# jdryg/vg-renderer

Measured on AMD Instinct MI355X. Metric: M tessellated verts/sec (stroke+fill AA), Tiger×10k batch, 1/2/4/8 GPUs, higher is better.
Workload: dtype f32; 1 GPU; tiger-like 240-path drawing (seed 2024) x 10000 instances per GPU: convexFillAA on every sub-path + polylineStrokeAA/AAThin (Butt/Miter) on 1/3 of the paths; instances_per_gpu=10000, draws_per_gpu=2400000, parallelism=shard1, verts_per_gpu=414940000, indices_per_gpu=1816170000, meshes_per_gpu=4350000, poly_verts_per_gpu=140430000

## Files before the change

### vg-renderer_amd/csrc/vgx_api.hip

```cpp
#include "vgx_internal.h"
#include "vgx_scan.h"
#include "vgx_scan_ops.h"
#include "vgx_pathsim.h"
#include "vgx_inst.h"
#include "vgx_flat1.h"
#include "vgx_thin.h"
#include "vgx_pathset_dev.h"
#include "vgx_tile.h"
#include "vgx_mscan.h"
#include "vgx_dash.h"
#include "vgx_update.h"
#include "vgx_raster.h"
#include "vgx_damage.h"
#include "vgx_pick.h"
#include "vgx_concave_lane.h"
#include "vgx_scratch.h"
#include <vector>
#include <algorithm>
#include <atomic>
#include <string.h>
#include <math.h>
#include <new>
#include <stdlib.h>

// ... 27 lines not shown
{
	T* host;
	uint32_t n;
	hipEvent_t ev;
	bool pending;
	int create(vgx_ctx* ctx, uint32_t count);
	void push(vgx_ctx* ctx, const void* dev, hipStream_t s);
	bool landed();
	void release();
};

struct VgxGatherWire { vgx_rank_sizes z; uint64_t chunk; };

struct VgxTemplateState
{
	bool on;
	bool isBatch;
	const vgx_pathset* ps;
	uint64_t psGen;
	uint32_t period;
	uint32_t classes;
	VgxTmplKernel kernel;
	uint32_t tileSize;
	vgx_sizes inst;
	vgx_sizes total;
	uint64_t numWg, nDraws;
	uint32_t round;
	uint32_t roundElems;
	uint32_t roundLds;
	uint64_t relemWords;
};
struct VgxTemplate : VgxTemplateState
{
	Buf<VgxTmplTile> tile;
	Buf<float2> poly; Buf<VgxTmplMesh> mesh; Buf<vgx_mesh> mtab; Buf<VgxTmplElem> elem; Buf<vgx_draw> draws;
	Buf<unsigned long long> hash, clsSum; Buf<uint32_t> instCls, clsRep; Buf<VgxTmplClass> cls; Buf<VgxTmplInst> iinfo; Buf<uint2> wg;
	Buf<VgxTmplRoundMesh> trmesh; Buf<uint2> tmsz;
	Buf<unsigned long long> rsz, itot, iplace; Buf<uint2> relem; Buf<VgxTmplMeshPlace> mplace;
};
static_assert(sizeof(VgxTmplWg) == sizeof(uint2) && offsetof(VgxTmplWg, inst) == offsetof(uint2, x) && offsetof(VgxTmplWg, tile) == offsetof(uint2, y), "the host's workgroup table is uploaded as uint2");
static_assert(sizeof(VgxTmplClass) == 40 && offsetof(VgxTmplClass, round) == 32 && sizeof(VgxTmplClass().round) == 8, "VgxTmplClass: the named words lie where the padding did");
static_assert(sizeof(VgxTmplMesh) == 64 && offsetof(VgxTmplMesh, fringe_bits) == 56 && offsetof(VgxTmplMesh, round_no) == 60, "VgxTmplMesh: the named words lie where the padding did");

struct vgx_ctx
{
	int device;
	int lastHipError;
	int pendingHipError;
	DevBufList scratch;
	Buf<uint32_t> asmJump0, asmJump1, asmStart, meshBase;
	vgx_assembly asmCfg;
	bool asmArmed;
	Buf<uint64_t> subPrefix;
	DevBuf cmdPrefix;
	DevBuf poly;
	DevBuf partial;
	Buf<uint32_t> cmdCnt, serialList;
	Buf<VgxSubRec> subFirst;
	Buf<float> leafOverflow;
// ... 1392 lines not shown
	if ((st = ensure(ctx, ctx->tmpl.relem, (classes ? ctx->tmpl.relemWords : n * a.num_round_elems) + 1)) != VGX_OK) { return st; }
	if ((st = ensure(ctx, ctx->tmpl.mplace, (classes ? a.total.num_meshes : n * a.inst.num_meshes) + 1)) != VGX_OK) { return st; }
	if ((st = ensure(ctx, ctx->partial, VGX_SCAN_BLOCKS * sizeof(Sum3))) != VGX_OK) { return st; }
	a.rsz = classes ? nullptr : ctx->tmpl.rsz.ptr(); a.relem = ctx->tmpl.relem.ptr();
	a.mplace = ctx->tmpl.mplace.ptr();
	if (vgx_tmpl_round_per_instance(a)) {
		if ((st = ensure(ctx, ctx->tmpl.itot, (n + 1) * 2)) != VGX_OK) { return st; }
		if ((st = ensure(ctx, ctx->tmpl.iplace, (n + 1) * 2)) != VGX_OK) { return st; }
		a.itot = ctx->tmpl.itot.ptr(); a.iplace = ctx->tmpl.iplace.ptr();
	}
	vgx_launch_tmpl_round_sizes(a, (Sum3*)ctx->partial.p, s);
	mark(ctx, s, "tmpl_round_sizes");
	return VGX_OK;
}

static void tmplArgs(vgx_ctx* ctx, const vgx_pathset* ps, const vgx_draw* draws, uint64_t ndraws, VgxTmplArgs& a)
{
	a.draws = draws; a.ndraws = ndraws; a.period = ctx->tmpl.period; a.ninst = ndraws / ctx->tmpl.period; a.npaths = ps->dev.npaths;
	a.tdraws = ctx->tmpl.draws.ptr(); a.tpoly = ctx->tmpl.poly.ptr(); a.tmesh = ctx->tmpl.mesh.ptr();
	a.tmtab = ctx->tmpl.mtab.ptr(); a.telem = ctx->tmpl.elem.ptr();
	a.inst = ctx->tmpl.inst;
	a.ttile = ctx->tmpl.tile.ptr();
	a.tile = ctx->tmpl.tileSize;
	a.tiles_per_inst = (uint32_t)((ctx->tmpl.inst.num_elements + a.tile - 1) / a.tile);
	a.caps = ctx->caps;
	a.totals = ctx->totals.ptr();
	a.kernel = ctx->tmpl.kernel;
	if (ctx->tmpl.classes > 1) {
		a.iinfo = ctx->tmpl.iinfo.ptr(); a.wg = ctx->tmpl.wg.ptr(); a.num_wg = ctx->tmpl.numWg;
		a.cls = ctx->tmpl.cls.ptr(); a.round_lds = ctx->tmpl.roundLds;
		a.total = ctx->tmpl.total;
	} else {
		memset(&a.total, 0, sizeof(a.total));
		vgx_tmpl_add_instances(a.total, a.ninst, ctx->tmpl.inst);
		a.num_wg = a.ninst * (uint64_t)a.tiles_per_inst;
	}
}

static int runTmpl(vgx_ctx* ctx, const vgx_pathset* ps, const vgx_draw* draws, uint64_t ndraws, const vgx_mesh_out* out, vgx_sizes* dev_sizes, uint32_t* dev_status, hipStream_t s)
{
	VgxTmplArgs a;
	memset(&a, 0, sizeof(a));
	tmplArgs(ctx, ps, draws, ndraws, a);
	a.pos = out->pos; a.color = out->color; a.idx = out->idx; a.meshes_out = out->meshes;
	a.caps.vertices = out->cap_vertices; a.caps.indices = out->cap_indices; a.caps.meshes = out->cap_meshes;
	if (a.num_wg > 0x7FFFFFFFull) { return VGX_E_RANGE; }
	noteHip(ctx, hipMemsetAsync(ctx->totals.p, 0, sizeof(VgxTotals), s));
// ... 157 lines not shown
	noteHip(ctx, hipMemsetAsync(ctx->tmpl.cls.p, 0, ((size_t)T + 1) * sizeof(VgxTmplClass), j.s));
	if (general) {
		j.b.mdesc = ctx->mdesc.ptr(); j.b.num_meshes = j.all.num_meshes; j.b.nclasses = T; j.b.cls = ctx->tmpl.cls.ptr();
		vgx_launch_tmpl_styles(j.b, j.s);
		HIPCHK(ctx, hipMemcpyAsync(&styles, &VGX_TMPL_STYLES(ctx->tmpl.cls.ptr(), T), sizeof(uint32_t), hipMemcpyDeviceToHost, j.s));
		HIPCHK(ctx, hipStreamSynchronize(j.s));
	}
	j.t.kernel = vgx_tmpl_kernel_for(styles);
	j.t.tileSize = vgx_tmpl_tile_for(j.t.kernel, ctx->optTmplTile);
	return VGX_OK;
}

static TmplStage tmplBuildTables(TmplJob& j)
{
	vgx_ctx* ctx = j.ctx;
	const uint32_t T = j.T;
	const uint64_t M = j.all.num_meshes, V = j.all.num_poly_vertices;
	VgxTmplBuild& b = j.b;
	int st;
	b.draws = ctx->tmpl.draws.ptr(); b.poly = (const float2*)ctx->poly.p; b.mdesc = ctx->mdesc.ptr(); b.mprep = ctx->mprep.ptr(); b.mtab = ctx->mtab.ptr();
	b.prefix_fill = ctx->elemPrefix.ptr(); b.prefix_stroke = ctx->elemPrefixS.ptr();
	b.num_meshes = M; b.num_elems = j.all.num_elements; b.tile = j.t.tileSize; b.period = (uint32_t)j.P; b.nclasses = T;
	b.num_vertices = j.all.num_vertices; b.num_indices = j.all.num_indices; b.cls = ctx->tmpl.cls.ptr();
	vgx_launch_tmpl_classes(b, j.s);
	j.cls.resize((size_t)T + 1);
	std::vector<unsigned long long> csum(((size_t)T + 1) * 5, 0ull);
	if (T > 1) {
		if ((st = ensure(ctx, ctx->tmpl.clsSum, ((size_t)T + 1) * 5)) != VGX_OK) { return st; }
		vgx_launch_tmpl_class_sums(b, ctx->dinfo.ptr(), (const uint64_t*)ctx->cmdPrefix.p, j.P * T, j.all, ctx->tmpl.clsSum.ptr(), j.s);
		HIPCHK(ctx, hipMemcpyAsync(csum.data(), ctx->tmpl.clsSum.p, csum.size() * sizeof(unsigned long long), hipMemcpyDeviceToHost, j.s));
	}
	HIPCHK(ctx, hipMemcpyAsync(j.cls.data(), ctx->tmpl.cls.p, ((size_t)T + 1) * sizeof(VgxTmplClass), hipMemcpyDeviceToHost, j.s));
	HIPCHK(ctx, hipStreamSynchronize(j.s));
	if (T > 1 && !vgx_tmpl_class_sizes(j.cls.data(), csum.data(), T, j.csz)) { return TMPL_ORDINARY; }
	const uint64_t tiles = j.cls[T].tile0;
	if ((st = ensure(ctx, ctx->tmpl.poly, V + 1)) != VGX_OK) { return st; }
	if ((st = ensure(ctx, ctx->tmpl.mesh, M + 1)) != VGX_OK) { return st; }
	if ((st = ensure(ctx, ctx->tmpl.mtab, M + 1)) != VGX_OK) { return st; }
	if ((st = ensure(ctx, ctx->tmpl.elem, tiles * j.t.tileSize + 64)) != VGX_OK) { return st; }
	if ((st = ensure(ctx, ctx->tmpl.tile, tiles + 1)) != VGX_OK) { return st; }
	if ((st = ensure(ctx, ctx->tmpl.trmesh, M + 2)) != VGX_OK) { return st; }
	if ((st = ensure(ctx, ctx->tmpl.tmsz, M + 1)) != VGX_OK) { return st; }
	if ((st = ensure(ctx, ctx->partial, VGX_SCAN_BLOCKS * sizeof(Sum3))) != VGX_OK) { return st; }
	b.tmsz = ctx->tmpl.tmsz.ptr(); b.trmesh = ctx->tmpl.trmesh.ptr();
	b.has_round = vgx_tmpl_kernel_is_round(j.t.kernel) ? 1u : 0u;
	b.partial = (Sum3*)ctx->partial.p;
	b.ttile = ctx->tmpl.tile.ptr();
	b.tmesh = ctx->tmpl.mesh.ptr(); b.tmtab = ctx->tmpl.mtab.ptr(); b.telem = ctx->tmpl.elem.ptr();
	vgx_launch_tmpl_build(b, j.s);
	HIPCHK(ctx, hipMemcpyAsync(ctx->tmpl.poly.p, ctx->poly.p, V * 2 * sizeof(float), hipMemcpyDeviceToDevice, j.s));
	return VGX_OK;
}

static TmplStage tmplReadRoundLayout(TmplJob& j)
{
	vgx_ctx* ctx = j.ctx;
	const uint32_t T = j.T;
	j.clsRelems.assign(T, 0);
// ... 1609 lines not shown
```

### vg-renderer_amd/csrc/vgx_internal.h

```cpp
#ifndef VGX_INTERNAL_H
#define VGX_INTERNAL_H

#include <hip/hip_runtime.h>
#include <stdint.h>
#include "../../include/vgx.h"
#include "vgx_lane.h"

#include "vgx_internal_types.h"
#include "vgx_tmpl_plan.h"

struct VgxFlattenArgs
{
	VgxPathSetDev ps;
	const vgx_draw* draws;
	uint64_t ndraws;
	const uint64_t* cmd_prefix;
	const uint64_t* sub_prefix;
	uint32_t* cmd_cnt;
	vgx_draw_info* dinfo;
	float* poly;
	vgx_subpath* subs;
	VgxMeshDesc* mdesc;
	VgxMeshPrep* mprep;
	vgx_mesh* mtab;
// ... 31 lines not shown
	vgx_mesh* meshes_out;
	const uint32_t* mesh_base;
	VgxTotals* totals;
	VgxCaps caps;
	int no_long;
	int tile_mode;
};


#ifndef VGX_TMPL_THREADS
#define VGX_TMPL_THREADS 512
#endif
struct VgxTmplBuild
{
	const vgx_draw* draws;
	const VgxMeshDesc* mdesc;
	const VgxMeshPrep* mprep;
	const vgx_mesh* mtab;
	const float2* poly;
	const uint64_t* prefix_fill;
	const uint64_t* prefix_stroke;
	uint64_t num_meshes, num_elems;
	uint32_t tile;
	VgxTmplMesh* tmesh;
	vgx_mesh* tmtab;
	VgxTmplElem* telem;
	VgxTmplTile* ttile;
	uint32_t period;
	uint32_t nclasses;
	uint64_t num_vertices, num_indices;
	VgxTmplClass* cls;
	VgxTmplRoundMesh* trmesh;
	uint2* tmsz;
	uint32_t has_round;
	struct Sum3* partial;
};
struct VgxTmplArgs
{
	const vgx_draw* draws;
	uint64_t ndraws;
	uint64_t ninst;
	uint32_t period;
	uint32_t npaths;
	const vgx_draw* tdraws;
	const float2* tpoly;
	const VgxTmplMesh* tmesh;
// ... 406 lines not shown
```

### vg-renderer_amd/csrc/vgx_tmpl.hip

```cpp
#include <stddef.h>
#include <type_traits>
#include "vgx_internal.h"
#include "vgx_wave.h"
#include "vgx_elem.h"
#include "vgx_tmpl_elem.h"
#include "vgx_scan_ops.h"

namespace {

static_assert(sizeof(vgx_draw) == 64 && offsetof(vgx_draw, path) == 0 && offsetof(vgx_draw, fill_flags) == 4 && offsetof(vgx_draw, fill_color) == 8
	&& offsetof(vgx_draw, stroke_flags) == 12 && offsetof(vgx_draw, stroke_color) == 16 && offsetof(vgx_draw, stroke_width) == 20 && offsetof(vgx_draw, scale) == 24
	&& offsetof(vgx_draw, tess_tol) == 28 && offsetof(vgx_draw, fringe) == 32 && offsetof(vgx_draw, mtx) == 36, "draw records are read as four 16-byte words");
__device__ __forceinline__ bool tmpl_same(const uint4 a0, const uint4 a1, const uint4 a2, const uint4 b0, const uint4 b1, const uint4 b2)
{
	return ((a0.x == b0.x) & (a0.y == b0.y) & (a0.w == b0.w) & (a1.y == b1.y) & (a1.z == b1.z) & (a1.w == b1.w) & (a2.x == b2.x)) != 0;
}

__device__ __forceinline__ uint32_t tmpl_validate(const uint4 q0, const uint4 q1, const uint4 q2, const uint4 q3, uint32_t npaths)
{
	const uint32_t sf = q0.w;
	if (q0.x >= npaths || ((sf & VGX_STROKE_ENABLE) && (VGX_STROKE_CAP(sf) > 2u || VGX_STROKE_JOIN(sf) > 2u))) { return VGX_E_INVALID_ARG; }
	const float sw = __uint_as_float(q1.y), sc = __uint_as_float(q1.z), tt = __uint_as_float(q1.w), fr = __uint_as_float(q2.x);
	const float m0 = __uint_as_float(q2.y), m1 = __uint_as_float(q2.z), m2 = __uint_as_float(q2.w);
	const float m3 = __uint_as_float(q3.x), m4 = __uint_as_float(q3.y), m5 = __uint_as_float(q3.z);
// ... 43 lines not shown
{
	for (uint64_t i = (uint64_t)blockIdx.x * blockDim.x + threadIdx.x; i < ndraws; i += (uint64_t)gridDim.x * blockDim.x) {
		const uint4* q = (const uint4*)(draws + i);
		const uint4 q0 = q[0], q1 = q[1], q2 = q[2];
		const uint64_t inst = i / P;
		unsigned long long h = tmpl_mix(0x243F6A8885A308D3ull, (uint32_t)(i - inst * P));
		h = tmpl_mix(h, q0.x); h = tmpl_mix(h, q0.y); h = tmpl_mix(h, q0.w); h = tmpl_mix(h, q1.y); h = tmpl_mix(h, q1.z); h = tmpl_mix(h, q1.w); h = tmpl_mix(h, q2.x);
		atomicAdd(&hashes[inst], h);
	}
}
__global__ __launch_bounds__(256) void k_tmpl_check_cls(const vgx_draw* draws, uint64_t ndraws, uint64_t P, const uint32_t* inst_cls, const uint32_t* cls_rep, VgxTotals* totals)
{
	bool bad = false;
	for (uint64_t i = (uint64_t)blockIdx.x * blockDim.x + threadIdx.x; i < ndraws; i += (uint64_t)gridDim.x * blockDim.x) {
		const uint64_t inst = i / P;
		const uint64_t k = i - inst * P;
		const uint4* q = (const uint4*)(draws + i);
		const uint4* t = (const uint4*)(draws + (uint64_t)cls_rep[inst_cls[inst]] * P + k);
		bad = bad || !tmpl_same(q[0], q[1], q[2], t[0], t[1], t[2]);
	}
	if (bad) { totals->tmpl_bad = 1u; }
}

__global__ void k_tmpl_classes(VgxTmplBuild B)
{
	const uint64_t M = B.num_meshes;
	uint32_t tile0 = 0;
	for (uint32_t c = 0; c <= B.nclasses; ++c) {
		uint64_t lo = 0, hi = M;
		const uint64_t d0 = (uint64_t)c * B.period;
		while (lo < hi) {
			const uint64_t mid = (lo + hi) >> 1;
			if (B.mdesc[mid].draw < d0) { lo = mid + 1; } else { hi = mid; }
		}
		VgxTmplClass r;
		r.mesh0 = (uint32_t)lo;
		r.elem0 = B.prefix_fill[lo] + B.prefix_stroke[lo];
		r.v0 = lo < M ? B.mtab[lo].first_vertex : B.num_vertices;
		r.i0 = lo < M ? B.mtab[lo].first_index : B.num_indices;
		r.tile0 = tile0;
		r.round[VGX_TC_ELEM0] = B.cls[c].round[VGX_TC_ELEM0]; r.round[VGX_TC_MESH0] = 0;
		B.cls[c] = r;
		if (c > 0) {
			const uint64_t e = r.elem0 - B.cls[c - 1].elem0;
			B.cls[c].tile0 = B.cls[c - 1].tile0 + (uint32_t)((e + B.tile - 1) / B.tile);
		}
		tile0 = B.cls[c].tile0;
	}
}
__global__ __launch_bounds__(256) void k_tmpl_class_sums(VgxTmplBuild B, const vgx_draw_info* dinfo, const uint64_t* cmdPrefix, uint64_t numDraws, vgx_sizes all, unsigned long long* sums)
{
	__shared__ unsigned long long s_serial;
	const uint32_t c = blockIdx.x;
	const uint64_t d0 = (uint64_t)c * B.period;
	if (threadIdx.x == 0) { s_serial = 0ull; }
	__syncthreads();
	if (c > 0) {
		unsigned long long n = 0;
		for (uint64_t d = d0 - B.period + threadIdx.x; d < d0; d += 256) { n += (dinfo[d].flags & 1u) ? 1ull : 0ull; }
		if (n) { atomicAdd(&s_serial, n); }
	}
	__syncthreads();
	if (threadIdx.x == 0) {
		unsigned long long* o = sums + 5ull * c;
		const bool end = d0 >= numDraws;
		o[0] = end ? all.num_poly_vertices : dinfo[d0].first_poly_vertex;
		o[1] = end ? all.num_subpaths : dinfo[d0].first_subpath;
		o[2] = cmdPrefix[end ? numDraws : d0];
// ... 114 lines not shown
	__shared__ unsigned long long s_poly[VGX_TMPL_ELEMS_MAXM];
	__shared__ uint32_t s_pick;
	__shared__ uint64_t s_b[6];
	auto lastLe = [&](uint64_t x, uint64_t lo, uint64_t hi) {
		while (hi - lo > 1) {
			const uint64_t step = (hi - lo + 255) / 256;
			const uint64_t m = lo + (uint64_t)tid * step;
			if (tid == 0) { s_pick = 0; }
			__syncthreads();
			if (tid > 0 && m < hi && first(m) <= x) { atomicMax(&s_pick, tid); }
			__syncthreads();
			const uint32_t k = s_pick;
			__syncthreads();
			lo += (uint64_t)k * step;
			hi = lo + step < hi ? lo + step : hi;
		}
		return lo;
	};
	for (uint64_t tile = blockIdx.x; tile < B.cls[B.nclasses].tile0; tile += gridDim.x) {
		uint32_t c = 0;
		while (c + 1 < B.nclasses && B.cls[c + 1].tile0 <= tile) { ++c; }
		const VgxTmplClass cl = B.cls[c];
		const uint64_t cEnd = B.cls[c + 1].elem0;
		const uint64_t x0 = cl.elem0 + (tile - cl.tile0) * T;
		const uint64_t x1 = x0 + T < cEnd ? x0 + T : cEnd;
		const uint64_t m0 = lastLe(x0, 0, M);
		const uint64_t m1 = x1 >= E ? M : lastLe(x1, m0, (m0 + T / 2 + 2 < M) ? m0 + T / 2 + 2 : M);
		const uint64_t hi = m1 < M ? m1 + 1 : M;
		const bool inLds = hi - m0 <= (uint64_t)VGX_TMPL_ELEMS_MAXM;
		__syncthreads();
		if (inLds) {
			for (uint64_t m = m0 + tid; m < hi; m += 256) {
				const VgxMeshDesc md = B.mdesc[m];
				s_pf[m - m0] = B.prefix_fill[m];
				s_ps[m - m0] = B.prefix_stroke[m] | (VGX_MD_KIND(md.kind) < VGX_MESH_STROKE ? (1ull << 63) : 0ull);
				s_poly[m - m0] = md.poly_first;
			}
		}
		if (tid == 0) {
			auto before = [&](uint64_t x, uint64_t m, uint64_t* fB, uint64_t* sB, uint32_t* j) {
				if (m >= M) { *fB = B.prefix_fill[M]; *sB = B.prefix_stroke[M]; *j = 0; return; }
				const uint64_t pf = B.prefix_fill[m], psk = B.prefix_stroke[m];
				const uint32_t jj = (uint32_t)(x - (pf + psk));
				const bool f = VGX_MD_KIND(B.mdesc[m].kind) < VGX_MESH_STROKE;
				*j = jj; *fB = pf + (f ? jj : 0u); *sB = psk + (f ? 0u : jj);
			};
			uint64_t f0, s0, f1, s1;
			uint32_t j0, j1;
			before(x0, m0, &f0, &s0, &j0);
			before(x1, x1 >= E ? M : m1, &f1, &s1, &j1);
// ... 230 lines not shown
	uint32_t cmesh0;
	const vgx_draw* tdraws;
};
__device__ __forceinline__ void tmpl_mesh_out(const VgxTmplArgs& A, const TmplPlace& P, uint32_t mesh)
{
	vgx_mesh mr = A.tmtab[mesh];
	mr.first_vertex += P.v;
	mr.first_index += P.i;
	mr.draw += P.draw0;
	A.meshes_out[P.m + (mesh - P.cmesh0)] = mr;
}

__device__ __forceinline__ void tmpl_mesh_out_placed(const VgxTmplArgs& A, const TmplPlace& P, uint32_t mesh, uint4 mi)
{
	vgx_mesh mr = A.tmtab[mesh];
	mr.first_vertex = P.v + mi.x;
	mr.first_index = P.i + mi.y;
	mr.num_vertices = mi.z;
	mr.num_indices = mi.w;
	mr.draw += P.draw0;
	A.meshes_out[P.m + (mesh - P.cmesh0)] = mr;
}

struct TmplVtx01
{
	float x0, y0, x1, y1;
	__device__ __forceinline__ V2 ld(uint32_t i) const { const bool z = i == 0; return v2(z ? x0 : x1, z ? y0 : y1); }
};

__device__ __forceinline__ void tmpl_stroke_counts(uint32_t kind, uint32_t cap, uint32_t join, uint32_t H, uint32_t* capNv, uint32_t* capNiFirst, uint32_t* joinNv, uint32_t* joinNi, uint32_t* bridge)
{
	const uint32_t R = (kind == VGX_MESH_STROKE) ? 2u : (kind == VGX_MESH_STROKE_AA ? 4u : 3u);
	*bridge = (R - 1) * 6;
	const bool roundCap = cap == VGX_CAP_ROUND && kind != VGX_MESH_STROKE_AA_THIN;
	if (roundCap) {
		*capNv = kind == VGX_MESH_STROKE_AA ? 2 * H : H;
		*capNiFirst = kind == VGX_MESH_STROKE_AA ? 9 * H - 12 : 3 * (H - 2);
	} else {
		*capNv = R;
		*capNiFirst = kind == VGX_MESH_STROKE_AA ? 6u : 0u;
	}
	if (kind == VGX_MESH_STROKE_AA_THIN) { const bool bevel = join != VGX_JOIN_MITER; *joinNv = bevel ? 4u : 3u; *joinNi = bevel ? 3u : 0u; }
	else if (join == VGX_JOIN_MITER) { *joinNv = R; *joinNi = 0; }
	else if (kind == VGX_MESH_STROKE_AA) { *joinNv = 6; *joinNi = 9; }
	else { *joinNv = 3; *joinNi = 3; }
}
// ... 298 lines not shown
	}
}
#ifndef VGX_TMPL_OCC
#define VGX_TMPL_OCC
#endif
#ifndef VGX_TMPL_G_THREADS
#define VGX_TMPL_G_THREADS 256
#endif
#define VGX_TMPL_G_TILE VGX_TMPL_GENERAL_TILE
template<int KIND, int THREADS, int MAXTILE, int ROUND = 0>
__device__ __forceinline__ void tmpl_emit_body(const VgxTmplArgs& A)
{
	constexpr bool GENERAL = KIND == 2;
	static_assert(ROUND == 0 || GENERAL || KIND == 3 || KIND == 4, "Round joins take the general element body, or -- closed AA strokes only -- tmpl_stroke_elem_round");
	constexpr int CH = MAXTILE / THREADS;
	__shared__ TmplDraw s_draw[VGX_TMPL_MAXM];
	__shared__ TmplRec s_rec[VGX_TMPL_MAXM];
	__shared__ float2 s_vtx[MAXTILE];
	__shared__ float2 s_dir[MAXTILE];
	__shared__ uint32_t s_status;
	__shared__ uint4 s_mi[ROUND ? VGX_TMPL_MAXM : 1];
	__shared__ float4 s_rmesh[ROUND ? VGX_TMPL_MAXM : 1];
	__shared__ float s_fringe[KIND >= 2 ? VGX_TMPL_MAXM : 1];
	const uint32_t tid = threadIdx.x;
	uint32_t inst32, t;
	TmplPlace P;
	uint64_t relemAt = 0;
	if (A.wg) {
		const uint2 w = A.wg[blockIdx.x];
		inst32 = w.x; t = w.y;
		const VgxTmplInst ii = A.iinfo[inst32];
		P.v = ii.v; P.i = ii.i; P.m = ii.m;
		if (ROUND) { P.v = A.iplace[2 * (uint64_t)inst32]; P.i = A.iplace[2 * (uint64_t)inst32 + 1]; relemAt = ii.rel; }
	} else {
		inst32 = blockIdx.x / A.tiles_per_inst;
		t = blockIdx.x - inst32 * A.tiles_per_inst;
		P.v = (uint64_t)inst32 * A.inst.num_vertices; P.i = (uint64_t)inst32 * A.inst.num_indices; P.m = (uint64_t)inst32 * A.inst.num_meshes;
		if (ROUND) {
			if (A.iplace) { P.v = A.iplace[2 * (uint64_t)inst32]; P.i = A.iplace[2 * (uint64_t)inst32 + 1]; }
			else { const VgxTmplMeshPlace* mp = A.mplace + (uint64_t)inst32 * A.inst.num_meshes; P.v = mp->v; P.i = mp->i; }
			relemAt = (uint64_t)inst32 * A.num_round_elems;
		}
	}
	const uint64_t inst = inst32;
	const VgxTmplTile tl = A.ttile[t];
	P.draw0 = (uint32_t)(inst * A.period); P.cmesh0 = tl.cmesh0; P.tdraws = A.tdraws + tl.cdraw0;
// ... 53 lines not shown
			} else if (j == 0 && A.meshes_out) { tmpl_mesh_out(A, P, er.mesh); }
			const uint32_t ibase = meshBase ? meshBase[er.mesh - P.cmesh0] : 0u;
			tmpl_elem_emit<KIND, 0>(O, j, tm.kind, N, vOff, iOff, ibase, kind < VGX_MESH_STROKE ? dr.fill_color : dr.stroke_color, f0, tm.f1, tmpl_xf(xf, vt[j]), dir(j), dir, vtx,
				__uint_as_float(tm.fringe_bits), P.tdraws + tm.drawk, A.tmesh + er.mesh, rpl);
		}
		return;
	}
#ifdef VGX_TMPL_PROFILE
	const unsigned long long tp0 = wall_clock64();
#define TMPL_PROF(i) do { if (tid == 0) { atomicAdd(&A.totals->prof[i], wall_clock64() - tp0); } } while (0)
#else
#define TMPL_PROF(i)
#endif
	if (ROUND && tid < nm) { s_mi[tid] = minfoOf(mA + tid); }
	VgxTmplElem er[CH];
	uint32_t rb[ROUND ? CH : 1], rk[ROUND ? CH : 1];
#pragma unroll
	for (int c = 0; c < CH; ++c) {
		const uint32_t s = (uint32_t)c * THREADS + tid;
		er[c].mesh = mA; er[c].jq = 0; er[c].lx = 0.0f; er[c].ly = 0.0f;
		if (s < nel) { er[c] = telem[s]; }
	}
	VgxTmplMesh tm;
	memset(&tm, 0, sizeof(tm));
	tm.n = 3; tm.drawk = dA; tm.kind = VGX_MESH_FILL;
	uint32_t ibase = 0;
	uint4 mi = make_uint4(0u, 0u, 0u, 0u);
	if (tid < nm) {
		tm = A.tmesh[mA + tid];
		if (meshBase) { ibase = meshBase[mA - P.cmesh0 + tid]; }
	}
	if (tid < nd) { s_draw[tid] = tmpl_load_draw(A, idraws, P.tdraws, dA + tid); }
	if (tid == 0) { s_status = A.totals->status; }
	__syncthreads();
	const uint32_t status = s_status;
	if (tid < nm) {
		if (ROUND) { mi = s_mi[tid]; tm.v_off = mi.x; tm.i_off = mi.y; }
		const uint32_t kind = VGX_MD_KIND(tm.kind);
		const TmplDraw* d = &s_draw[tm.drawk - dA];
		TmplRec r;
		r.ibase = ibase; r.n = tm.n; r.v_off = tm.v_off; r.i_off = tm.i_off;
		r.kind = (tm.kind & 0xFFFFu) | ((tm.drawk - dA) << 16); r.color = kind < VGX_MESH_STROKE ? d->fill_color : d->stroke_color; r.f0 = tm.f0; r.f1 = tm.f1;
		if (KIND >= 2) { s_fringe[tid] = __uint_as_float(tm.fringe_bits); }
		if (ROUND) {
			const bool rj = tm.round_no != 0;
			s_rmesh[tid] = make_float4(__uint_as_float(mi.z), __uint_as_float(mi.w), rj ? tm.l2[0] : 0.0f, rj ? tm.l2[1] : __uint_as_float(~0u));
		}
		if (kind == VGX_MESH_FILL_AA) { r.f0 = tmpl_fill_aa(tmpl_draw_xf(d), make_float2(tm.l0[0], tm.l0[1]), make_float2(tm.l1[0], tm.l1[1]), make_float2(tm.l2[0], tm.l2[1]), tm.f0); }
		s_rec[tid] = r;
		if ((tid > 0 || firstWhole) && A.meshes_out && status == VGX_OK) {
			if (ROUND) { tmpl_mesh_out_placed(A, P, mA + tid, mi); } else { tmpl_mesh_out(A, P, mA + tid); }
		}
	}
	__syncthreads();
	TMPL_PROF(0);
	if (status != VGX_OK) {
		return;
	}
	if (ROUND) {
#pragma unroll
		for (int c = 0; c < CH; ++c) {
			const uint32_t s = (uint32_t)c * THREADS + tid;
			rb[c] = ~0u; rk[c] = 0;
			if (s < nel) {
				const uint32_t e0 = __float_as_uint(s_rmesh[er[c].mesh - mA].w);
				if (e0 != ~0u) {
					const uint2* w = relemOf(e0 + (er[c].jq & 0xFFFFu));
					if (GENERAL) { const uint2 bk = *w; rb[c] = bk.x; rk[c] = bk.y; } else { rb[c] = w->x; }
				}
			}
		}
	}
	V2 p1[CH];
#pragma unroll
	for (int c = 0; c < CH; ++c) {
// ... 7 lines not shown
	}
	__syncthreads();
	TMPL_PROF(1);
	auto vtxAt = [&](uint32_t mesh, const TmplRec* rp, int q0, uint32_t jj) {
		const uint32_t qq = (uint32_t)(q0 + (int)jj);
		if (qq < nel) { const float2 v = s_vtx[qq]; return v2(v.x, v.y); }
		return tmpl_xf(tmpl_draw_xf(&s_draw[TMPL_REC_DK(rp)]), A.tpoly[A.tmesh[mesh].poly_first + jj]);
	};
	V2 d12[CH];
#pragma unroll
	for (int c = 0; c < CH; ++c) {
		const uint32_t s = (uint32_t)c * THREADS + tid;
		d12[c] = v2(0.0f, 0.0f);
		if (s < nel) {
			const TmplRec* rp = &s_rec[er[c].mesh - mA];
			const uint32_t j = er[c].jq & 0xFFFFu, N = rp->n;
			const int q0 = (int)(er[c].jq >> 16) - (int)j;
			d12[c] = v2dir(p1[c], vtxAt(er[c].mesh, rp, q0, j + 1 < N ? j + 1 : 0u));
			s_dir[er[c].jq >> 16] = make_float2(d12[c].x, d12[c].y);
		}
	}
	__syncthreads();
	TMPL_PROF(2);
	auto element = [&](auto passTag, uint32_t s, const VgxTmplElem& e, V2 pv, V2 dv, bool placed, uint32_t wx, uint32_t wy) {
		TmplRoundPlace rpl;
		rpl.placed = placed;
		tmpl_round_unword(wx, wy, &rpl.b, &rpl.k, &rpl.nvPrev, &rpl.prevInner);
		rpl.nv = 0; rpl.ni = 0; rpl.da = 0.0f;
		if (s < nel) {
			const uint32_t mesh = e.mesh;
			const TmplRec* rp = &s_rec[mesh - mA];
			const uint32_t j = e.jq & 0xFFFFu, N = rp->n;
			const int q0 = (int)(e.jq >> 16) - (int)j;
			auto dir = [&](uint32_t jj) {
				const uint32_t qq = (uint32_t)(q0 + (int)jj);
				if (qq < nel) { const float2 v = s_dir[qq]; return v2(v.x, v.y); }
				return v2dir(vtxAt(mesh, rp, q0, jj), vtxAt(mesh, rp, q0, jj + 1 < N ? jj + 1 : 0u));
			};
			auto vtx = [&](uint32_t jj) { return vtxAt(mesh, rp, q0, jj); };
			const float fringe = KIND >= 2 ? s_fringe[mesh - mA] : 0.0f;
			if (ROUND && placed) { const float4 rm = s_rmesh[mesh - mA]; rpl.nv = __float_as_uint(rm.x); rpl.ni = __float_as_uint(rm.y); rpl.da = rm.z; }
			const vgx_draw* tdraw = P.tdraws;
			if (GENERAL && decltype(passTag)::value == 2) { tdraw = P.tdraws + (dA + TMPL_REC_DK(rp)); }
			tmpl_elem_emit<KIND, decltype(passTag)::value>(O, j, rp->kind & 0xFFFFu, N, rp->v_off, rp->i_off, rp->ibase, rp->color, rp->f0, rp->f1, pv, dv, dir, vtx, fringe, tdraw, A.tmesh + mesh,
				rpl);
		}
	};
// ... 388 lines not shown
void vgx_launch_tmpl_check(const vgx_draw* draws, uint64_t ndraws, uint32_t npaths, VgxTotals* totals, hipStream_t s)
{
	hipLaunchKernelGGL(k_tmpl_check, dim3(1024), dim3(256), 0, s, draws, ndraws, npaths, totals);
}

void vgx_launch_tmpl_hash(const vgx_draw* draws, uint64_t ndraws, uint64_t period, unsigned long long* hashes, hipStream_t s)
{
	hipLaunchKernelGGL(k_tmpl_hash, dim3(1024), dim3(256), 0, s, draws, ndraws, period, hashes);
}

void vgx_launch_tmpl_check_cls(const vgx_draw* draws, uint64_t ndraws, uint64_t period, const uint32_t* inst_cls, const uint32_t* cls_rep, VgxTotals* totals, hipStream_t s)
{
	hipLaunchKernelGGL(k_tmpl_check_cls, dim3(1024), dim3(256), 0, s, draws, ndraws, period, inst_cls, cls_rep, totals);
}

void vgx_launch_tmpl_styles(const VgxTmplBuild& b, hipStream_t s)
{
	const uint64_t gm = (b.num_meshes + 255) / 256;
	if (b.num_meshes) { hipLaunchKernelGGL(k_tmpl_styles, dim3((unsigned)(gm > 1024 ? 1024 : gm)), dim3(256), 0, s, b); }
}

void vgx_launch_tmpl_classes(const VgxTmplBuild& b, hipStream_t s)
{
	hipLaunchKernelGGL(k_tmpl_classes, dim3(1), dim3(1), 0, s, b);
}

void vgx_launch_tmpl_class_sums(const VgxTmplBuild& b, const vgx_draw_info* dinfo, const uint64_t* cmdPrefix, uint64_t numDraws, const vgx_sizes& all, unsigned long long* sums, hipStream_t s)
{
	hipLaunchKernelGGL(k_tmpl_class_sums, dim3(b.nclasses + 1), dim3(256), 0, s, b, dinfo, cmdPrefix, numDraws, all, sums);
}

void vgx_launch_tmpl_build(const VgxTmplBuild& b, hipStream_t s)
{
	const uint64_t gm = (b.num_meshes + 255) / 256;
	const uint64_t nt = (b.num_elems + b.tile - 1) / b.tile + b.nclasses;
	if (b.num_meshes) {
		hipLaunchKernelGGL(k_tmpl_meshes, dim3((unsigned)(gm > 4096 ? 4096 : gm)), dim3(256), 0, s, b);
		if (b.has_round) {
			OpTmplRoundIndex op; op.B = b; vgx_device_scan(op, b.partial, s, b.num_meshes);
			if (b.nclasses > 1) { hipLaunchKernelGGL(k_tmpl_round_classes, dim3(1), dim3(1), 0, s, b); }
		}
	}
	if (b.num_elems) {
		hipLaunchKernelGGL(k_tmpl_elems, dim3((unsigned)(nt > 65536 ? 65536 : nt)), dim3(256), 0, s, b);
		hipLaunchKernelGGL(k_tmpl_tiles, dim3((unsigned)((nt + 255) / 256)), dim3(256), 0, s, b);
	}
}

void vgx_launch_tmpl_mtab(const VgxTmplArgs& a, vgx_mesh* mtab, VgxMeshDesc* mdesc, hipStream_t s)
{
	hipLaunchKernelGGL(k_tmpl_mtab, dim3(2048), dim3(256), 0, s, a, mtab, mdesc);
}

void vgx_launch_tmpl_emit(const VgxTmplArgs& a, hipStream_t s)
{
	const uint64_t blocks = a.wg ? a.num_wg : a.ninst * a.tiles_per_inst;
	if (!blocks) { return; }
	const dim3 grid((unsigned)blocks);
// ... 11 lines not shown
```

### vg-renderer_amd/csrc/vgx_tmpl_plan.h

```cpp
#ifndef VGX_TMPL_PLAN_H
#define VGX_TMPL_PLAN_H

#include <stdint.h>
#include <string.h>
#include <stddef.h>
#include <vector>
#include <unordered_map>
#include "vgx_internal_types.h"

#ifndef VGX_TMPL_MAX_TILE
#define VGX_TMPL_MAX_TILE 2048
#endif
#ifndef VGX_TMPL_RC_TILE
#define VGX_TMPL_RC_TILE 2048
#endif
#ifndef VGX_TMPL_GENERAL_TILE
#define VGX_TMPL_GENERAL_TILE 2048
#endif

enum VgxTmplStyle : uint32_t
{
	VGX_TS_OPEN_MITER = 1u,
	VGX_TS_OTHER = 2u,
	VGX_TS_ROUND = 4u,
// ... 8 lines not shown
	VGX_TK_GENERAL = 2,
	VGX_TK_ROUND = 3,
	VGX_TK_BEVEL = 4,
	VGX_TK_ROUND_AA = 5,
	VGX_TK_ROUND_AA_OPEN = 6
};

inline VgxTmplKernel vgx_tmpl_kernel_for(uint32_t styles)
{
	if (styles & VGX_TS_ROUND) {
		if (styles & (VGX_TS_OPEN_MITER | VGX_TS_OTHER)) { return VGX_TK_ROUND; }
		return (styles & VGX_TS_ROUND_AA_OPEN) ? VGX_TK_ROUND_AA_OPEN : VGX_TK_ROUND_AA;
	}
	if (styles & VGX_TS_OTHER) { return VGX_TK_GENERAL; }
	if (styles & VGX_TS_CLOSED_BEVEL) { return (styles & VGX_TS_OPEN_MITER) ? VGX_TK_GENERAL : VGX_TK_BEVEL; }
	return (styles & VGX_TS_OPEN_MITER) ? VGX_TK_OPEN : VGX_TK_EMIT;
}
inline bool vgx_tmpl_kernel_is_round(VgxTmplKernel k) { return k == VGX_TK_ROUND || k == VGX_TK_ROUND_AA || k == VGX_TK_ROUND_AA_OPEN; }
inline uint32_t vgx_tmpl_tile_for(VgxTmplKernel k, uint32_t optTile)
{
	if ((k == VGX_TK_GENERAL || k == VGX_TK_ROUND) && optTile > VGX_TMPL_GENERAL_TILE) { return (uint32_t)VGX_TMPL_GENERAL_TILE; }
	if ((k == VGX_TK_ROUND_AA || k == VGX_TK_ROUND_AA_OPEN) && optTile == VGX_TMPL_MAX_TILE) { return VGX_TMPL_RC_TILE; }
	return optTile;
}

inline bool vgx_tmpl_eligible(const VgxTotals& ht, bool roundOk)
{
	const vgx_sizes& z = ht.sizes;
	return !((ht.num_round_meshes && !roundOk) || z.num_elements == 0 || z.num_elements >= (1ull << 31) || z.num_vertices >= (1ull << 29)
		|| z.num_indices >= (1ull << 31) || z.num_poly_vertices >= (1ull << 32) || z.num_meshes >= (1ull << 32));
}

inline bool vgx_tmpl_group_classes(const unsigned long long* hashes, uint64_t ninst, std::vector<uint32_t>& instCls, std::vector<uint32_t>& reps)
{
	instCls.assign((size_t)ninst, 0u);
	reps.clear();
	std::unordered_map<unsigned long long, uint32_t> seen;
	for (uint64_t k = 0; k < ninst; ++k) {
		const auto it = seen.find(hashes[k]);
		uint32_t c;
		if (it != seen.end()) { c = it->second; }
		else {
			c = (uint32_t)reps.size();
			if (c == VGX_TMPL_MAX_CLASSES) { return false; }
			seen.emplace(hashes[k], c);
			reps.push_back((uint32_t)k);
// ... 101 lines not shown
```

Before: 255,500 M verts/s.

## Snap template tile boundaries to mesh starts and defer mesh-table writes

Result: faster. 277,000 M verts/s, median of 6 (+8.4%).

```diff
diff --git a/vg-renderer_amd/csrc/vgx_api.hip b/vg-renderer_amd/csrc/vgx_api.hip
--- a/vg-renderer_amd/csrc/vgx_api.hip
+++ b/vg-renderer_amd/csrc/vgx_api.hip
@@ -73,6 +73,7 @@
 	uint32_t classes;
 	VgxTmplKernel kernel;
 	uint32_t tileSize;
+	uint32_t tilesPerInst;
 	vgx_sizes inst;
 	vgx_sizes total;
 	uint64_t numWg, nDraws;
@@ -85,7 +86,7 @@
 {
 	Buf<VgxTmplTile> tile;
 	Buf<float2> poly; Buf<VgxTmplMesh> mesh; Buf<vgx_mesh> mtab; Buf<VgxTmplElem> elem; Buf<vgx_draw> draws;
-	Buf<unsigned long long> hash, clsSum; Buf<uint32_t> instCls, clsRep; Buf<VgxTmplClass> cls; Buf<VgxTmplInst> iinfo; Buf<uint2> wg;
+	Buf<unsigned long long> hash, clsSum; Buf<uint32_t> instCls, clsRep; Buf<VgxTmplClass> cls; Buf<uint32_t> clsLmax; Buf<uint64_t> tbound; Buf<VgxTmplInst> iinfo; Buf<uint2> wg;
 	Buf<VgxTmplRoundMesh> trmesh; Buf<uint2> tmsz;
 	Buf<unsigned long long> rsz, itot, iplace; Buf<uint2> relem; Buf<VgxTmplMeshPlace> mplace;
 };
@@ -1524,7 +1525,7 @@
 	a.inst = ctx->tmpl.inst;
 	a.ttile = ctx->tmpl.tile.ptr();
 	a.tile = ctx->tmpl.tileSize;
-	a.tiles_per_inst = (uint32_t)((ctx->tmpl.inst.num_elements + a.tile - 1) / a.tile);
+	a.tiles_per_inst = ctx->tmpl.tilesPerInst;
 	a.caps = ctx->caps;
 	a.totals = ctx->totals.ptr();
 	a.kernel = ctx->tmpl.kernel;
@@ -1728,6 +1729,11 @@
 	b.prefix_fill = ctx->elemPrefix.ptr(); b.prefix_stroke = ctx->elemPrefixS.ptr();
 	b.num_meshes = M; b.num_elems = j.all.num_elements; b.tile = j.t.tileSize; b.period = (uint32_t)j.P; b.nclasses = T;
 	b.num_vertices = j.all.num_vertices; b.num_indices = j.all.num_indices; b.cls = ctx->tmpl.cls.ptr();
+	if ((st = ensure(ctx, ctx->tmpl.clsLmax, (size_t)T + 1)) != VGX_OK) { return st; }
+	noteHip(ctx, hipMemsetAsync(ctx->tmpl.clsLmax.p, 0, ((size_t)T + 1) * sizeof(uint32_t), j.s));
+	b.lmax = ctx->tmpl.clsLmax.ptr();
+	if ((st = ensure(ctx, ctx->tmpl.tbound, (size_t)vgx_tmpl_max_tiles(j.all.num_elements, j.t.tileSize, T) + 1)) != VGX_OK) { return st; }
+	b.tbound = ctx->tmpl.tbound.ptr();
 	vgx_launch_tmpl_classes(b, j.s);
 	j.cls.resize((size_t)T + 1);
 	std::vector<unsigned long long> csum(((size_t)T + 1) * 5, 0ull);
@@ -1740,6 +1746,7 @@
 	HIPCHK(ctx, hipStreamSynchronize(j.s));
 	if (T > 1 && !vgx_tmpl_class_sizes(j.cls.data(), csum.data(), T, j.csz)) { return TMPL_ORDINARY; }
 	const uint64_t tiles = j.cls[T].tile0;
+	j.t.tilesPerInst = j.cls[1].tile0;
 	if ((st = ensure(ctx, ctx->tmpl.poly, V + 1)) != VGX_OK) { return st; }
 	if ((st = ensure(ctx, ctx->tmpl.mesh, M + 1)) != VGX_OK) { return st; }
 	if ((st = ensure(ctx, ctx->tmpl.mtab, M + 1)) != VGX_OK) { return st; }
diff --git a/vg-renderer_amd/csrc/vgx_internal.h b/vg-renderer_amd/csrc/vgx_internal.h
--- a/vg-renderer_amd/csrc/vgx_internal.h
+++ b/vg-renderer_amd/csrc/vgx_internal.h
@@ -77,6 +77,8 @@
 	const uint64_t* prefix_stroke;
 	uint64_t num_meshes, num_elems;
 	uint32_t tile;
+	uint32_t* lmax;
+	uint64_t* tbound;
 	VgxTmplMesh* tmesh;
 	vgx_mesh* tmtab;
 	VgxTmplElem* telem;
diff --git a/vg-renderer_amd/csrc/vgx_tmpl.hip b/vg-renderer_amd/csrc/vgx_tmpl.hip
--- a/vg-renderer_amd/csrc/vgx_tmpl.hip
+++ b/vg-renderer_amd/csrc/vgx_tmpl.hip
@@ -89,6 +89,21 @@
 	if (bad) { totals->tmpl_bad = 1u; }
 }
 
+__global__ __launch_bounds__(256) void k_tmpl_mesh_lmax(VgxTmplBuild B)
+{
+	uint32_t cur = 0, best = 0;
+	for (uint64_t m = (uint64_t)blockIdx.x * blockDim.x + threadIdx.x; m < B.num_meshes; m += (uint64_t)gridDim.x * blockDim.x) {
+		const uint32_t c = B.mdesc[m].draw / B.period;
+		const uint64_t len = (B.prefix_fill[m + 1] + B.prefix_stroke[m + 1]) - (B.prefix_fill[m] + B.prefix_stroke[m]);
+		if (c != cur) {
+			if (best) { atomicMax(&B.lmax[cur], best); }
+			cur = c; best = 0;
+		}
+		const uint32_t l = vgx_tmpl_snap_len(len, B.tile);
+		best = l > best ? l : best;
+	}
+	if (best) { atomicMax(&B.lmax[cur], best); }
+}
 __global__ void k_tmpl_classes(VgxTmplBuild B)
 {
 	const uint64_t M = B.num_meshes;
@@ -110,7 +125,27 @@
 		B.cls[c] = r;
 		if (c > 0) {
 			const uint64_t e = r.elem0 - B.cls[c - 1].elem0;
-			B.cls[c].tile0 = B.cls[c - 1].tile0 + (uint32_t)((e + B.tile - 1) / B.tile);
+			uint64_t nt = vgx_tmpl_tile_count(e, vgx_tmpl_stride(B.tile, B.lmax[c - 1]));
+			const uint64_t mLo = B.cls[c - 1].mesh0, mHi = r.mesh0;
+			if (vgx_tmpl_greedy_class(mHi - mLo, e, B.tile)) {
+				uint64_t* tb = B.tbound + B.cls[c - 1].tile0;
+				uint64_t b = B.cls[c - 1].elem0;
+				nt = 0;
+				while (b < r.elem0) {
+					tb[nt++] = b;
+					const uint64_t nom = vgx_tmpl_greedy_nominal(b, r.elem0, B.tile);
+					if (nom >= r.elem0) { break; }
+					uint64_t lo2 = mLo, hi2 = mHi;
+					while (hi2 - lo2 > 1) {
+						const uint64_t mid = (lo2 + hi2) >> 1;
+						if (B.prefix_fill[mid] + B.prefix_stroke[mid] <= nom) { lo2 = mid; } else { hi2 = mid; }
+					}
+					const uint64_t f0 = B.prefix_fill[lo2] + B.prefix_stroke[lo2], f1 = B.prefix_fill[lo2 + 1] + B.prefix_stroke[lo2 + 1];
+					b = vgx_tmpl_snap_boundary(nom, f0, f1 - f0, B.tile);
+				}
+				B.lmax[c - 1] |= 0x80000000u;
+			}
+			B.cls[c].tile0 = B.cls[c - 1].tile0 + (uint32_t)nt;
 		}
 		tile0 = B.cls[c].tile0;
 	}
@@ -271,10 +306,15 @@
 		while (c + 1 < B.nclasses && B.cls[c + 1].tile0 <= tile) { ++c; }
 		const VgxTmplClass cl = B.cls[c];
 		const uint64_t cEnd = B.cls[c + 1].elem0;
-		const uint64_t x0 = cl.elem0 + (tile - cl.tile0) * T;
-		const uint64_t x1 = x0 + T < cEnd ? x0 + T : cEnd;
-		const uint64_t m0 = lastLe(x0, 0, M);
-		const uint64_t m1 = x1 >= E ? M : lastLe(x1, m0, (m0 + T / 2 + 2 < M) ? m0 + T / 2 + 2 : M);
+		const uint32_t S = vgx_tmpl_stride((uint32_t)T, B.lmax[c] & 0x7FFFFFFFu);
+		const bool greedy = (B.lmax[c] >> 31) != 0;
+		const uint64_t n0 = greedy ? B.tbound[tile] : vgx_tmpl_nominal_boundary(cl.elem0, cEnd, tile - cl.tile0, S);
+		const uint64_t n1 = greedy ? (tile + 1 < B.cls[c + 1].tile0 ? B.tbound[tile + 1] : cEnd) : vgx_tmpl_nominal_boundary(cl.elem0, cEnd, tile - cl.tile0 + 1, S);
+		auto len = [&](uint64_t m) { return first(m + 1) - first(m); };
+		const uint64_t m0 = lastLe(n0, 0, M);
+		const uint64_t x0 = vgx_tmpl_snap_boundary(n0, first(m0), len(m0), (uint32_t)T);
+		const uint64_t m1 = n1 >= E ? M : lastLe(n1, m0, (m0 + T / 2 + 2 < M) ? m0 + T / 2 + 2 : M);
+		const uint64_t x1 = m1 >= M ? n1 : vgx_tmpl_snap_boundary(n1, first(m1), len(m1), (uint32_t)T);
 		const uint64_t hi = m1 < M ? m1 + 1 : M;
 		const bool inLds = hi - m0 <= (uint64_t)VGX_TMPL_ELEMS_MAXM;
 		__syncthreads();
@@ -551,6 +591,20 @@
 	A.meshes_out[P.m + (mesh - P.cmesh0)] = mr;
 }
 
+static_assert(sizeof(vgx_mesh) == 32 && offsetof(vgx_mesh, num_vertices) == 16 && offsetof(vgx_mesh, num_indices) == 20 && offsetof(vgx_mesh, subpath_kind) == 28, "the words read below");
+__device__ __forceinline__ uint2 tmpl_mesh_sizes(const VgxTmplArgs& A, uint32_t mesh) { return *(const uint2*)&A.tmtab[mesh].num_vertices; }
+__device__ __forceinline__ void tmpl_mesh_out_parts(const VgxTmplArgs& A, const TmplPlace& P, uint32_t mesh, uint32_t vOff, uint32_t iOff, uint32_t nv, uint32_t ni, uint32_t drawk, uint32_t subpathKind)
+{
+	vgx_mesh mr;
+	mr.first_vertex = P.v + vOff;
+	mr.first_index = P.i + iOff;
+	mr.num_vertices = nv;
+	mr.num_indices = ni;
+	mr.draw = drawk + P.draw0;
+	mr.subpath_kind = subpathKind;
+	A.meshes_out[P.m + (mesh - P.cmesh0)] = mr;
+}
+
 struct TmplVtx01
 {
 	float x0, y0, x1, y1;
@@ -895,6 +949,8 @@
 	__shared__ uint4 s_mi[ROUND ? VGX_TMPL_MAXM : 1];
 	__shared__ float4 s_rmesh[ROUND ? VGX_TMPL_MAXM : 1];
 	__shared__ float s_fringe[KIND >= 2 ? VGX_TMPL_MAXM : 1];
+	__shared__ uint2 s_msz[VGX_TMPL_MAXM];
+	__shared__ uint32_t s_msub[VGX_TMPL_MAXM];
 	const uint32_t tid = threadIdx.x;
 	uint32_t inst32, t;
 	TmplPlace P;
@@ -994,15 +1050,20 @@
 		if (s < nel) { er[c] = telem[s]; }
 	}
 	VgxTmplMesh tm;
-	memset(&tm, 0, sizeof(tm));
-	tm.n = 3; tm.drawk = dA; tm.kind = VGX_MESH_FILL;
+	tm.poly_first = 0; tm.n = 3; tm.v_off = 0; tm.i_off = 0; tm.drawk = dA; tm.kind = VGX_MESH_FILL; tm.f0 = 0.0f; tm.f1 = 0.0f;
+	tm.l0[0] = 0.0f; tm.l0[1] = 0.0f; tm.l1[0] = 0.0f; tm.l1[1] = 0.0f; tm.l2[0] = 0.0f; tm.l2[1] = 0.0f; tm.fringe_bits = 0; tm.round_no = 0;
 	uint32_t ibase = 0;
 	uint4 mi = make_uint4(0u, 0u, 0u, 0u);
+	const bool meshOut = tid < nm && (tid > 0 || firstWhole) && A.meshes_out;
+	uint2 msz = make_uint2(0u, 0u);
+	uint32_t msub = 0;
 	if (tid < nm) {
 		tm = A.tmesh[mA + tid];
 		if (meshBase) { ibase = meshBase[mA - P.cmesh0 + tid]; }
 	}
+	if (meshOut) { msz = tmpl_mesh_sizes(A, mA + tid); msub = A.tmtab[mA + tid].subpath_kind; }
 	if (tid < nd) { s_draw[tid] = tmpl_load_draw(A, idraws, P.tdraws, dA + tid); }
+	if (meshOut) { s_msz[tid] = msz; s_msub[tid] = msub; }
 	if (tid == 0) { s_status = A.totals->status; }
 	__syncthreads();
 	const uint32_t status = s_status;
@@ -1020,9 +1081,6 @@
 		}
 		if (kind == VGX_MESH_FILL_AA) { r.f0 = tmpl_fill_aa(tmpl_draw_xf(d), make_float2(tm.l0[0], tm.l0[1]), make_float2(tm.l1[0], tm.l1[1]), make_float2(tm.l2[0], tm.l2[1]), tm.f0); }
 		s_rec[tid] = r;
-		if ((tid > 0 || firstWhole) && A.meshes_out && status == VGX_OK) {
-			if (ROUND) { tmpl_mesh_out_placed(A, P, mA + tid, mi); } else { tmpl_mesh_out(A, P, mA + tid); }
-		}
 	}
 	__syncthreads();
 	TMPL_PROF(0);
@@ -1076,7 +1134,13 @@
 	}
 	__syncthreads();
 	TMPL_PROF(2);
-	auto element = [&](auto passTag, uint32_t s, const VgxTmplElem& e, V2 pv, V2 dv, bool placed, uint32_t wx, uint32_t wy) {
+	if (meshOut) {
+		const TmplRec* r = &s_rec[tid];
+		uint2 z = s_msz[tid];
+		if (ROUND) { const uint4 q = s_mi[tid]; z = make_uint2(q.z, q.w); }
+		tmpl_mesh_out_parts(A, P, mA + tid, r->v_off, r->i_off, z.x, z.y, dA + TMPL_REC_DK(r), s_msub[tid]);
+	}
+	auto element =[&](auto passTag, uint32_t s, const VgxTmplElem& e, V2 pv, V2 dv, bool placed, uint32_t wx, uint32_t wy) {
 		TmplRoundPlace rpl;
 		rpl.placed = placed;
 		tmpl_round_unword(wx, wy, &rpl.b, &rpl.k, &rpl.nvPrev, &rpl.prevInner);
@@ -1511,6 +1575,8 @@
 
 void vgx_launch_tmpl_classes(const VgxTmplBuild& b, hipStream_t s)
 {
+	const uint64_t gm = (b.num_meshes + 255) / 256;
+	if (b.num_meshes) { hipLaunchKernelGGL(k_tmpl_mesh_lmax, dim3((unsigned)(gm > 1024 ? 1024 : gm)), dim3(256), 0, s, b); }
 	hipLaunchKernelGGL(k_tmpl_classes, dim3(1), dim3(1), 0, s, b);
 }
 
@@ -1522,7 +1588,7 @@
 void vgx_launch_tmpl_build(const VgxTmplBuild& b, hipStream_t s)
 {
 	const uint64_t gm = (b.num_meshes + 255) / 256;
-	const uint64_t nt = (b.num_elems + b.tile - 1) / b.tile + b.nclasses;
+	const uint64_t nt = vgx_tmpl_max_tiles(b.num_elems, b.tile, b.nclasses);
 	if (b.num_meshes) {
 		hipLaunchKernelGGL(k_tmpl_meshes, dim3((unsigned)(gm > 4096 ? 4096 : gm)), dim3(256), 0, s, b);
 		if (b.has_round) {
diff --git a/vg-renderer_amd/csrc/vgx_tmpl_plan.h b/vg-renderer_amd/csrc/vgx_tmpl_plan.h
--- a/vg-renderer_amd/csrc/vgx_tmpl_plan.h
+++ b/vg-renderer_amd/csrc/vgx_tmpl_plan.h
@@ -54,6 +54,42 @@
 	if ((k == VGX_TK_GENERAL || k == VGX_TK_ROUND) && optTile > VGX_TMPL_GENERAL_TILE) { return (uint32_t)VGX_TMPL_GENERAL_TILE; }
 	if ((k == VGX_TK_ROUND_AA || k == VGX_TK_ROUND_AA_OPEN) && optTile == VGX_TMPL_MAX_TILE) { return VGX_TMPL_RC_TILE; }
 	return optTile;
+}
+
+#if defined(__HIPCC__)
+#define VGX_TMPL_HD __host__ __device__
+#else
+#define VGX_TMPL_HD
+#endif
+VGX_TMPL_HD inline uint32_t vgx_tmpl_snap_limit(uint32_t T) { return T / 8u; }
+VGX_TMPL_HD inline uint32_t vgx_tmpl_snap_len(uint64_t meshLen, uint32_t T) { return meshLen <= (uint64_t)vgx_tmpl_snap_limit(T) ? (uint32_t)meshLen : 0u; }
+VGX_TMPL_HD inline uint32_t vgx_tmpl_stride(uint32_t T, uint32_t lmax) { return T - ((lmax ? lmax : 1u) - 1u); }
+VGX_TMPL_HD inline uint64_t vgx_tmpl_tile_count(uint64_t classElems, uint32_t stride) { return (classElems + stride - 1) / stride; }
+VGX_TMPL_HD inline uint64_t vgx_tmpl_nominal_boundary(uint64_t elem0, uint64_t end, uint64_t k, uint32_t stride)
+{
+	const uint64_t b = elem0 + k * (uint64_t)stride;
+	return b < end ? b : end;
+}
+VGX_TMPL_HD inline uint64_t vgx_tmpl_snap_boundary(uint64_t nominal, uint64_t meshFirst, uint64_t meshLen, uint32_t T)
+{
+	return (meshFirst < nominal && meshLen <= (uint64_t)vgx_tmpl_snap_limit(T)) ? meshFirst : nominal;
+}
+#ifndef VGX_TMPL_GREEDY_MAX_MESHES
+#define VGX_TMPL_GREEDY_MAX_MESHES 4096u
+#endif
+#define VGX_TMPL_GREEDY_MAX_TILES 64u
+VGX_TMPL_HD inline bool vgx_tmpl_greedy_class(uint64_t classMeshes, uint64_t classElems, uint32_t T)
+{
+	return classMeshes <= VGX_TMPL_GREEDY_MAX_MESHES && classElems <= (uint64_t)VGX_TMPL_GREEDY_MAX_TILES * (T - vgx_tmpl_snap_limit(T));
+}
+VGX_TMPL_HD inline uint64_t vgx_tmpl_greedy_nominal(uint64_t start, uint64_t end, uint32_t T)
+{
+	const uint64_t b = start + T;
+	return b < end ? b : end;
+}
+VGX_TMPL_HD inline uint64_t vgx_tmpl_max_tiles(uint64_t elems, uint32_t T, uint32_t nclasses)
+{
+	return elems / vgx_tmpl_stride(T, vgx_tmpl_snap_limit(T)) + nclasses + 1;
 }
 
 inline bool vgx_tmpl_eligible(const VgxTotals& ht, bool roundOk)
```
